# ufukpage/TripleD-Exploring-Depth-Estimation-with-Self-Supervised-Representation-Learning

Measured on AMD Instinct MI355X. Metric: train imgs/sec at KITTI 192x640 bs=12/GPU, higher is better.
Workload: dtype bf16 convs (MFMA) + f32 loss kernels

## Files before the change

### include/tripled_hip.h

```cpp
#ifndef TRIPLED_HIP_H
#define TRIPLED_HIP_H

#include <stddef.h>
#include <stdint.h>

#ifdef __cplusplus
extern "C" {
#endif

#define TD_ABI_VERSION 3
#define TD_MAX_SRC 4

#define TD_OK 0
#define TD_ERR_BAD_ARG (-1)
#define TD_ERR_UNSUPPORTED (-2)
#define TD_ERR_LAUNCH (-3)
#define TD_ERR_WORKSPACE (-4)

typedef void* td_stream_t;

int td_abi_version(void);
const char* td_error_string(int code);
const char* td_last_hip_error(void);

// ... 53 lines not shown

int td_maxpool5_fwd(const void* in, int dtype, int N, int H, int W, int C, void* out, uint8_t* idx,
                    td_stream_t stream);
int td_maxpool5_bwd(const void* grad_out, const uint8_t* idx, int dtype, int N, int H, int W, int C,
                    void* grad_in, td_stream_t stream);
int td_maxpool5_bwd_add(const void* grad_out, const uint8_t* idx, const void* add, int dtype, int N, int H, int W, int C,
                        void* grad_in, td_stream_t stream);

int td_maxpool3s2_fwd(const void* in, int dtype, int N, int H, int W, int C, void* out, uint8_t* idx,
                      td_stream_t stream);
int td_maxpool3s2_bwd(const void* grad_out, const uint8_t* idx, int dtype, int N, int H, int W, int C,
                      void* grad_in, td_stream_t stream);

int td_join_fwd(const void* a, const void* b, const void* tail, int dtype, long long npix, int C0, int C1, int C2,
                void* out, td_stream_t stream);
int td_join_bwd(const void* grad_out, int dtype, long long npix, int C0, int C1, int C2, void* grad_a, void* grad_b,
                void* grad_tail, td_stream_t stream);
int td_join_up2_fwd(const void* a, const void* b_half, const void* tail, int dtype, int N, int H, int W, int C0, int C1,
                    int C2, void* out, td_stream_t stream);
int td_join_up2_bwd(const void* grad_out, int dtype, int N, int H, int W, int C0, int C1, int C2, void* grad_a,
                    void* grad_b_half, void* grad_tail, td_stream_t stream);

long long td_bn_workspace_floats(long long M, int groups, int C);
int td_bn_fwd(const void* x, const void* residual, int dtype, const float* gamma, const float* beta,
              float* running_mean, float* running_var, float momentum, float eps, int relu, long long M, int groups,
              int C, void* y, float* save_mean, float* save_invstd, float* workspace, td_stream_t stream);
int td_bn_bwd(const void* dy, const void* x, const void* y, int dtype, const float* gamma, const float* beta, const float* save_mean,
              const float* save_invstd, int relu, long long M, int groups, int C, void* dx, void* dresidual,
              float* dgamma, float* dbeta, float* workspace, td_stream_t stream);

int td_conv1x1_stat_rows(long long M, int groups, int N);
int td_conv1x1_fwd(const void* x, const void* w, long long M, int groups, int K, int N, int Hi, int Wi, int stride, void* y,
                   float* stat_partials, td_stream_t stream);
int td_conv3x3_fwd(const void* x, const void* w, int B, int groups, int Hi, int Wi, int Cin, int N, int stride, int pad, void* y,
                   float* stat_partials, td_stream_t stream);
long long td_conv3x3_wgrad_workspace_floats(int B, int Ho, int Wo, int C, int N);
int td_conv3x3_wgrad(const void* dy, const void* x, int B, int Ho, int Wo, int C, int N, int pad, int dw_dtype, void* dw,
                     float* workspace, td_stream_t stream);
long long td_conv1x1_wgrad_workspace_floats(long long M, int K, int N);
int td_conv1x1_wgrad(const void* dy, const void* x, long long M, int K, int N, int Hi, int Wi, int stride, int dw_dtype, void* dw,
                     float* workspace, td_stream_t stream);
int td_conv1x1_wgrad_group(int n, const void* const* dy, const void* const* x, const long long* M, const int* K, const int* N,
                           const int* Hi, const int* Wi, const int* stride, const int* dw_dtype, void* const* dw,
                           float* const* workspace, td_stream_t stream);
int td_bn_fwd_from_partials(const void* x, const void* residual, int dtype, const float* gamma, const float* beta,
                            float* running_mean, float* running_var, float momentum, float eps, int relu, long long M,
                            int groups, int C, float* partials, int stat_rows, void* y, float* save_mean,
                            float* save_invstd, td_stream_t stream);

long long td_bias_act_workspace_floats(long long M, int C);
int td_bias_act_fwd(const void* y, const void* bias, int bias_dtype, int dtype, long long M, int C, int act, void* a, td_stream_t stream);
int td_bias_act_bwd(const void* g, const void* a, int dtype, long long M, int C, int act, void* gy, void* dbias, int dbias_dtype,
                    float* workspace, td_stream_t stream);

int td_adam_flat(float* w, const float* grad, float* exp_avg, float* exp_avg_sq, void* lowp, long long n, long long n_lowp,
                 const float* step, const float* lr_dev, float lr_host, double beta1, double beta2, float eps, const float* total_norm,
                 float max_norm, td_stream_t stream);

int td_gather_flat(const void* const* srcs, const long long* dst_offsets, const long long* numels, int n, int src_dtype, float* flat,
                   td_stream_t stream);

int td_bn_partial_rows(long long M, int groups, int C);
int td_bn_fwd_partials(const void* x, int dtype, long long M, int groups, int C, float* partials, td_stream_t stream);
int td_bn_bwd_partials(const void* dy, const void* x, const void* y, int dtype, const float* gamma, const float* beta,
                       const float* save_mean, const float* save_invstd, int relu, long long M, int groups, int C, float* partials,
                       td_stream_t stream);
int td_bn_bwd_from_partials(const void* dy, const void* x, const void* y, int dtype, const float* gamma, const float* beta,
                            const float* save_mean, const float* save_invstd, int relu, long long M, int groups, int C,
                            float* partials, int stat_rows, void* dx, void* dresidual, float* dgamma, float* dbeta,
                            td_stream_t stream);
int td_conv1x1_fwd_bnrelu(const void* z, const void* w, long long M, int groups, int K, int N, float* in_partials, int in_rows,
                          const float* gamma, const float* beta, float* running_mean, float* running_var, float momentum, float eps,
                          float* save_mean, float* save_invstd, void* a_side, void* y, float* stat_partials, td_stream_t stream);
int td_conv1x1_dgrad(const void* dy, const void* w, long long M, int groups, int Cout, int Cin, const void* residual, void* dx,
                     td_stream_t stream);
int td_conv1x1_fwd_sum(const void* x, const void* w, long long M, int K, int N, const void* run_in, void* y, void* run_out,
                       td_stream_t stream);
int td_conv1x1_dgrad_bnsums(const void* dy, const void* w, long long M, int groups, int Cout, int Cin, const void* z,
                            const float* gamma, const float* beta, const float* save_mean, const float* save_invstd, void* dx,
                            float* out_partials, td_stream_t stream);
int td_conv1x1_dgrad_bnbwd(const void* g, const void* z, const void* w, long long M, int groups, int Cout, int Cin, float* in_partials,
                           int in_rows, const float* gamma, const float* beta, const float* save_mean, const float* save_invstd,
                           float* dgamma, float* dbeta, void* dz_side, const void* residual, void* dx, td_stream_t stream);

int td_bn_sync_fwd_sums(const void* x, int dtype, long long M, int groups, int C, float* sums, float* workspace,
                        td_stream_t stream);
int td_bn_sync_fwd_apply(const void* x, const void* residual, int dtype, const float* sums, const float* count,
                         const float* gamma, const float* beta, float* running_mean, float* running_var, float momentum,
                         float eps, int relu, long long M, int groups, int C, void* y, float* save_mean,
                         float* save_invstd, td_stream_t stream);
int td_bn_sync_bwd_sums(const void* dy, const void* x, const void* y, int dtype, const float* gamma, const float* beta,
                        const float* save_mean, const float* save_invstd, int relu, long long M, int groups, int C,
                        float* sums, float* workspace, td_stream_t stream);
int td_bn_sync_bwd_dx(const void* dy, const void* x, const void* y, int dtype, const float* local_sums,
                      const float* global_sums, const float* count, const float* gamma, const float* beta,
                      const float* save_mean, const float* save_invstd, int relu, long long M, int groups, int C,
                      void* dx, void* dresidual, float* dgamma, float* dbeta, float* coef, td_stream_t stream);

int td_edge_weights(const float* img, int B, int h, int w, float a, const float* scale6, float* Wt,
                    td_stream_t stream);
int td_featreg_num_blocks(int B, int h, int w, int C);
int td_featreg_fwd(const void* feat, int dtype, const float* Wt, int B, int h, int w, int C,
                   float* partial, td_stream_t stream);
int td_featreg_bwd(const void* feat, int dtype, const float* Wt, const float* gscale, int B, int h, int w,
                   int C, void* grad, td_stream_t stream);

// ... 139 lines not shown
```

### tripled-exploring-depth-estimation-with-self-supervised-representation-learning_amd/csrc/td_biasact.hip

```cpp
#include <hip/hip_bf16.h>

#include "td_common.h"
#include "td_vec8.h"

namespace td {

template <int ACT>
__device__ __forceinline__ float ba_fwd(float z) {
  if (ACT == 1) return z > 0.f ? z : expm1f(z);
  if (ACT == 2) return z > 0.f ? z : 0.01f * z;
  return z;
}
template <int ACT>
__device__ __forceinline__ float ba_bwd(float g, float a) {
  if (ACT == 1) return a > 0.f ? g : g * (a + 1.f);
  if (ACT == 2) return a > 0.f ? g : 0.01f * g;
  return g;
}

template <typename T, int ACT>
__global__ __launch_bounds__(TD_THREADS) void bias_act_fwd_kernel(const T* __restrict__ y, const void* __restrict__ bias, int bias_bf16,
                                                                  long long nvec, int cvec, T* __restrict__ a) {
  const long long stride = (long long)gridDim.x * TD_THREADS;
  long long i = (long long)blockIdx.x * TD_THREADS + threadIdx.x;
  const int cg = (int)(i % cvec);
  float b[8];
#pragma unroll
  for (int e = 0; e < 8; ++e)
    b[e] = !bias ? 0.f : bias_bf16 ? bf2f(reinterpret_cast<const unsigned short*>(bias)[cg * 8 + e]) : reinterpret_cast<const float*>(bias)[cg * 8 + e];
  for (; i < nvec; i += stride) {
    float v[8];
    load8(y + i * 8, v);
#pragma unroll
    for (int e = 0; e < 8; ++e) v[e] = ba_fwd<ACT>(v[e] + b[e]);
    store8(a + i * 8, v);
  }
}

template <typename T, int ACT>
__global__ __launch_bounds__(TD_THREADS) void bias_act_bwd_kernel(const T* __restrict__ g, const T* __restrict__ a, long long nvec, int cvec,
                                                                  T* __restrict__ gy, float* __restrict__ partial) {
  __shared__ float red[TD_THREADS][9];
  const long long stride = (long long)gridDim.x * TD_THREADS;
  long long i = (long long)blockIdx.x * TD_THREADS + threadIdx.x;
  float s[8];
#pragma unroll
  for (int e = 0; e < 8; ++e) s[e] = 0.f;
  for (; i < nvec; i += stride) {
    float vg[8], va[8];
    load8(g + i * 8, vg);
    if (ACT != 0) load8(a + i * 8, va);
#pragma unroll
    for (int e = 0; e < 8; ++e) {
      vg[e] = ba_bwd<ACT>(vg[e], ACT != 0 ? va[e] : 0.f);
      s[e] += vg[e];
    }
    if (ACT != 0) store8(gy + i * 8, vg);
  }
#pragma unroll
  for (int e = 0; e < 8; ++e) red[threadIdx.x][e] = s[e];
  __syncthreads();
  const int C = cvec * 8;
  if ((int)threadIdx.x < C) {
    const int c = threadIdx.x, cg = c >> 3, e = c & 7;
    float t = 0.f;
    for (int j = cg; j < TD_THREADS; j += cvec) t += red[j][e];
    partial[(size_t)blockIdx.x * C + c] = t;
  }
}

template <typename T>
// ... 79 lines not shown
```

### tripled-exploring-depth-estimation-with-self-supervised-representation-learning_amd/hostside/mono/model/networks.py

```python
import os

import numpy as np
import torch
import torch.nn as nn
import torch.nn.functional as F



FUSED_BN_OFF = bool(os.environ.get("TD_NO_FUSED_BN"))


def _ops():
    from tripled_amd import ops
    return ops


def _dense_cl(x):
    if x.is_cuda and x.dim() == 4 and x.shape[1] % 8 == 0 and x.dtype in (torch.float32, torch.bfloat16) \
            and not x.is_contiguous(memory_format=torch.channels_last) and x.stride(1) == 1:
        return x.contiguous(memory_format=torch.channels_last)
    return x


def _fell_back(site, x, why=""):
# ... 506 lines not shown
            y = F.conv2d(x, w, b)
        ctx.save_for_backward(x, w)
        ctx.has_bias = b is not None
        return y

    @staticmethod
    def backward(ctx, gy):
        x, w = ctx.saved_tensors
        with torch.backends.cudnn.flags(enabled=True, benchmark=False):
            gx, gw, gb = torch.ops.aten.convolution_backward(gy, x, w, [w.shape[0]] if ctx.has_bias else None, [1, 1], [0, 0], [1, 1],
                                                              False, [0, 0], 1, [True, True, ctx.has_bias])
        return gx, gw, (gb if ctx.has_bias else None)


class _KeepChannels(torch.autograd.Function):

    @staticmethod
    def forward(ctx, y, c):
        ctx.pad = y.shape[1] - c
        return y.narrow(1, 0, c)

    @staticmethod
    def backward(ctx, g):
        return F.pad(g, (0, 0, 0, 0, 0, ctx.pad)), None


FUSED_BIAS_ACT_OFF = bool(os.environ.get("TD_NO_FUSED_BIAS_ACT"))
FUSED_CRP_OFF = bool(os.environ.get("TD_NO_FUSED_CRP"))


def _activate(y, act):
    if act == "elu":
        return F.elu(y, inplace=True)
    if act == "leaky_relu":
        return F.leaky_relu(y)
    return y


def _conv2d_guarded(x, w, b, act=None):
    if x.is_cuda and x.shape[1] <= 16 and w.shape[0] <= 16 and x.shape[3] > 1024 and torch.backends.cudnn.benchmark:
        if torch.is_autocast_enabled():
            dt = torch.get_autocast_dtype("cuda")
            x, w, b = x.to(dt), w.to(dt), (b.to(dt) if b is not None else None)
        return _activate(_ConvImmediate.apply(x, w, b), act)
    if (act is not None or b is not None) and x.is_cuda and not FUSED_BIAS_ACT_OFF and torch.is_grad_enabled() \
            and torch.is_autocast_enabled() and torch.get_autocast_dtype("cuda") == torch.bfloat16:
        xb = x if x.dtype == torch.bfloat16 else x.to(torch.bfloat16)
        wb = w if w.dtype == torch.bfloat16 else w.to(torch.bfloat16)
        if _ops().conv_bias_act_supported(xb, wb, b, act):
            return _ops().conv_bias_act(xb, wb, b, act)
    return _activate(F.conv2d(x, w, b), act)


class Conv3x3(nn.Module):

    def __init__(self, in_channels, out_channels, use_refl=True):
        super().__init__()
        self.use_refl = use_refl
        self.pad = nn.ReflectionPad2d(1) if use_refl else nn.ZeroPad2d(1)
        self.conv = nn.Conv2d(int(in_channels), int(out_channels), 3)

    def _pad_input(self, x):
        x = _dense_cl(x)
        if self.use_refl and x.shape[1] % 8 == 0 and x.dtype in (torch.float32, torch.bfloat16) \
                and x.is_contiguous(memory_format=torch.channels_last) and x.shape[2] >= 2 and x.shape[3] >= 2:
            from tripled_amd import ops
            return ops.reflpad1(x)
        if self.use_refl:
            _fell_back("Conv3x3.pad", x)
        return self.pad(x)

    def forward(self, x, act=None):
        low_precision = x.is_cuda and (x.dtype == torch.bfloat16 or torch.is_autocast_enabled())
        if not low_precision or os.environ.get("TD_NO_CHANNEL_PAD"):
            return _activate(self.conv(self._pad_input(x) if x.is_cuda else self.pad(x)), act)
        w, b = self.conv.weight, self.conv.bias
        cout, cin = w.shape[0], w.shape[1]
        cin_p, cout_p = _round8(cin), _round8(cout)
        if cin_p == cin and cout_p == cout and x.shape[1] == cin:
            return _conv2d_guarded(self._pad_input(x), w, b, act)
        if x.shape[1] == cin and cin_p != cin:
            x = torch.cat((x, x.new_zeros(x.shape[0], cin_p - cin, x.shape[2], x.shape[3])), 1)
        if x.shape[1] != cin_p:
            raise ValueError("Conv3x3 expects %d (or pre-padded %d) input channels, got %d" % (cin, cin_p, x.shape[1]))
        if not x.is_contiguous(memory_format=torch.channels_last):
            x = x.contiguous(memory_format=torch.channels_last)
        w = F.pad(w, (0, 0, 0, 0, 0, cin_p - cin, 0, cout_p - cout))
        if b is not None and cout_p != cout:
            b = F.pad(b, (0, cout_p - cout))
        if cout_p != cout:
            return _activate(_KeepChannels.apply(_conv2d_guarded(self._pad_input(x), w, b), cout), act)
        return _conv2d_guarded(self._pad_input(x), w, b, act)

    def forward_up(self, x, act=None):
        w, b = self.conv.weight, self.conv.bias
        cout, cin = w.shape[0], w.shape[1]
        x = _dense_cl(x)
        low_precision = x.is_cuda and (x.dtype == torch.bfloat16 or torch.is_autocast_enabled())
        if (self.use_refl and x.is_cuda and x.shape[1] == cin and cin % 8 == 0 and (cout % 8 == 0 or low_precision)
                and x.dtype in (torch.float32, torch.bfloat16) and x.is_contiguous(memory_format=torch.channels_last)
                and not os.environ.get("TD_NO_FUSED_UPSAMPLE")):
            cout_p = _round8(cout)
            if cout_p != cout:
                w = F.pad(w, (0, 0, 0, 0, 0, 0, 0, cout_p - cout))
                b = F.pad(b, (0, cout_p - cout)) if b is not None else None
            if cout_p != cout:
                return _activate(_KeepChannels.apply(_conv2d_guarded(_ops().up2_reflpad1(x), w, b), cout), act)
            return _conv2d_guarded(_ops().up2_reflpad1(x), w, b, act)
        _fell_back("Conv3x3.forward_up", x)
        return self.forward(upsample(x), act)


class Conv5x5(nn.Module):
    def __init__(self, in_channels, out_channels, use_refl=True):
        super().__init__()
        self.pad = nn.ReflectionPad2d(2) if use_refl else nn.ZeroPad2d(2)
        self.conv = nn.Conv2d(int(in_channels), int(out_channels), 5)

    def forward(self, x):
        return self.conv(self.pad(x))


class ConvBlock(nn.Module):
    def __init__(self, in_channels, out_channels):
        super().__init__()
        self.conv = Conv3x3(in_channels, out_channels)
        self.nonlin = nn.ELU(inplace=True)

    def forward(self, x):
        return self.conv(x, act="elu")

    def forward_up(self, x):
        return self.conv.forward_up(x, act="elu")


class CRPBlock(nn.Module):

    def __init__(self, in_planes, out_planes, n_stages):
        super().__init__()
        for i in range(n_stages):
            setattr(self, "{}_{}".format(i + 1, "pointwise"),
                    Conv1x1(in_planes if i == 0 else out_planes, out_planes, False))
        self.stride = 1
        self.n_stages = n_stages
        self.maxpool = nn.MaxPool2d(kernel_size=5, stride=1, padding=2)

    def _pool(self, t):
        if t.is_cuda and t.is_contiguous(memory_format=torch.channels_last) and t.shape[1] % 8 == 0 \
                and t.dtype in (torch.float32, torch.bfloat16):
            from tripled_amd import ops
            return ops.maxpool5(t)
        _fell_back("CRPBlock.maxpool", t)
        return self.maxpool(t)

    def _fused(self, x):
        if FUSED_CRP_OFF or _FP8_1X1[0] or not (self.training and x.is_cuda and torch.is_grad_enabled()):
            return None
        if not (torch.is_autocast_enabled() and torch.get_autocast_dtype("cuda") == torch.bfloat16):
            return None
        convs = [getattr(self, "{}_{}".format(i + 1, "pointwise")).conv for i in range(self.n_stages)]
        if any(c.bias is not None for c in convs):
# ... 204 lines not shown
```

### tripled-exploring-depth-estimation-with-self-supervised-representation-learning_amd/native.py

```python
import ctypes
import os

import torch

from . import dispatch

_HERE = os.path.dirname(os.path.abspath(__file__))
LIB_PATH = os.path.join(_HERE, "lib", "libtripled_hip.so")

TD_MAX_SRC = 4

_PTRARR = ctypes.POINTER(ctypes.c_void_p)
_I, _F, _P = ctypes.c_int, ctypes.c_float, ctypes.c_void_p
_LLARR = ctypes.POINTER(ctypes.c_longlong)
_IARR = ctypes.POINTER(ctypes.c_int)
ABI_VERSION = 3

SIGNATURES = {
    "td_abi_version": (_I, []),
    "td_error_string": (ctypes.c_char_p, [_I]),
    "td_last_hip_error": (ctypes.c_char_p, []),
    "td_photo_num_blocks": (_I, [_I, _I, _I]),
    "td_photo_bwd_num_blocks": (_I, [_I, _I, _I]),
    "td_photo_identity": (_I, [_P, _PTRARR, _I, _I, _I, _I, _P, _P, _PTRARR, _P]),
    "td_photo_fwd": (_I, [_P, _PTRARR, _I, _P, _P, _P, _P, _P, _I, _I, _I, _I, _I, _F, _F, _P, _P, _P, _P, _P, _P]),
    "td_photo_bwd": (_I, [_P, _PTRARR, _P, _PTRARR, _I, _P, _P, _P, _P, _P, _I, _P, _F, _I, _I, _I, _I, _I, _F, _F, _P, _P, _P]),
    "td_pack_rgbx": (_I, [_P, _I, _I, _I, _P, _P]),
    "td_upsample_adjoint": (_I, [_P, _I, _I, _I, _I, _I, _P, _I, _P]),
    "td_upsample_adjoint_planes": (_I, [_P, _I, _I, _I, _I, _I, _I, _P, _I, _P]),
    "td_reduce_dP": (_I, [_P, _I, _I, _I, _I, _P, _P]),
    "td_sum_scaled": (_I, [_P, _I, _F, _P, _P]),
    "td_area_downsample": (_I, [_P, _I, _I, _I, _I, _I, _I, _P, _P]),
    "td_smooth_num_blocks": (_I, [_I, _I, _I]),
    "td_smooth_fwd": (_I, [_P, _P, _I, _I, _I, _I, _P, _P, _P]),
    "td_smooth_finish": (_I, [_P, _I, _I, _I, _F, _P, _P]),
    "td_smooth_bwd": (_I, [_P, _P, _P, _I, _I, _I, _I, _P, _F, _P, _P, _P, _I, _P]),
    "td_maxpool5_fwd": (_I, [_P, _I, _I, _I, _I, _I, _P, _P, _P]),
    "td_maxpool5_bwd": (_I, [_P, _P, _I, _I, _I, _I, _I, _P, _P]),
    "td_maxpool5_bwd_add": (_I, [_P, _P, _P, _I, _I, _I, _I, _I, _P, _P]),
    "td_conv1x1_fwd_sum": (_I, [_P, _P, ctypes.c_longlong, _I, _I, _P, _P, _P, _P]),
    "td_maxpool3s2_fwd": (_I, [_P, _I, _I, _I, _I, _I, _P, _P, _P]),
    "td_maxpool3s2_bwd": (_I, [_P, _P, _I, _I, _I, _I, _I, _P, _P]),
    "td_join_fwd": (_I, [_P, _P, _P, _I, ctypes.c_longlong, _I, _I, _I, _P, _P]),
    "td_join_bwd": (_I, [_P, _I, ctypes.c_longlong, _I, _I, _I, _P, _P, _P, _P]),
    "td_join_up2_fwd": (_I, [_P, _P, _P, _I, _I, _I, _I, _I, _I, _I, _P, _P]),
    "td_join_up2_bwd": (_I, [_P, _I, _I, _I, _I, _I, _I, _I, _P, _P, _P, _P]),
    "td_bn_workspace_floats": (ctypes.c_longlong, [ctypes.c_longlong, _I, _I]),
    "td_bn_fwd": (_I, [_P, _P, _I, _P, _P, _P, _P, _F, _F, _I, ctypes.c_longlong, _I, _I, _P, _P, _P, _P, _P]),
    "td_conv1x1_stat_rows": (_I, [ctypes.c_longlong, _I, _I]),
    "td_conv1x1_fwd": (_I, [_P, _P, ctypes.c_longlong, _I, _I, _I, _I, _I, _I, _P, _P, _P]),
    "td_conv3x3_fwd": (_I, [_P, _P, _I, _I, _I, _I, _I, _I, _I, _I, _P, _P, _P]),
    "td_conv3x3_wgrad_workspace_floats": (ctypes.c_longlong, [_I, _I, _I, _I, _I]),
    "td_conv3x3_wgrad": (_I, [_P, _P, _I, _I, _I, _I, _I, _I, _I, _P, _P, _P]),
    "td_conv1x1_wgrad_workspace_floats": (ctypes.c_longlong, [ctypes.c_longlong, _I, _I]),
    "td_conv1x1_wgrad": (_I, [_P, _P, ctypes.c_longlong, _I, _I, _I, _I, _I, _I, _P, _P, _P]),
    "td_conv1x1_wgrad_group": (_I, [_I, _PTRARR, _PTRARR, _LLARR, _IARR, _IARR, _IARR, _IARR, _IARR, _IARR, _PTRARR, _PTRARR, _P]),
    "td_bn_fwd_from_partials": (_I, [_P, _P, _I, _P, _P, _P, _P, _F, _F, _I, ctypes.c_longlong, _I, _I, _P, _I, _P, _P, _P, _P]),
    "td_bias_act_workspace_floats": (ctypes.c_longlong, [ctypes.c_longlong, _I]),
    "td_bias_act_fwd": (_I, [_P, _P, _I, _I, ctypes.c_longlong, _I, _I, _P, _P]),
    "td_bias_act_bwd": (_I, [_P, _P, _I, ctypes.c_longlong, _I, _I, _P, _P, _I, _P, _P]),
    "td_gather_flat": (_I, [_PTRARR, _LLARR, _LLARR, _I, _I, _P, _P]),
    "td_adam_flat": (_I, [_P, _P, _P, _P, _P, ctypes.c_longlong, ctypes.c_longlong, _P, _P, _F, ctypes.c_double, ctypes.c_double, _F, _P, _F, _P]),
    "td_bn_partial_rows": (_I, [ctypes.c_longlong, _I, _I]),
    "td_bn_fwd_partials": (_I, [_P, _I, ctypes.c_longlong, _I, _I, _P, _P]),
    "td_bn_bwd_partials": (_I, [_P, _P, _P, _I, _P, _P, _P, _P, _I, ctypes.c_longlong, _I, _I, _P, _P]),
    "td_bn_bwd_from_partials": (_I, [_P, _P, _P, _I, _P, _P, _P, _P, _I, ctypes.c_longlong, _I, _I, _P, _I, _P, _P, _P, _P, _P]),
    "td_conv1x1_fwd_bnrelu": (_I, [_P, _P, ctypes.c_longlong, _I, _I, _I, _P, _I, _P, _P, _P, _P, _F, _F, _P, _P, _P, _P, _P, _P]),
    "td_conv1x1_dgrad": (_I, [_P, _P, ctypes.c_longlong, _I, _I, _I, _P, _P, _P]),
    "td_conv1x1_dgrad_bnsums": (_I, [_P, _P, ctypes.c_longlong, _I, _I, _I, _P, _P, _P, _P, _P, _P, _P, _P]),
    "td_conv1x1_dgrad_bnbwd": (_I, [_P, _P, _P, ctypes.c_longlong, _I, _I, _I, _P, _I, _P, _P, _P, _P, _P, _P, _P, _P, _P, _P]),
    "td_bn_bwd": (_I, [_P, _P, _P, _I, _P, _P, _P, _P, _I, ctypes.c_longlong, _I, _I, _P, _P, _P, _P, _P, _P]),
    "td_edge_weights": (_I, [_P, _I, _I, _I, _F, ctypes.POINTER(ctypes.c_float), _P, _P]),
    "td_featreg_num_blocks": (_I, [_I, _I, _I, _I]),
    "td_featreg_fwd": (_I, [_P, _I, _P, _I, _I, _I, _I, _P, _P]),
    "td_featreg_bwd": (_I, [_P, _I, _P, _P, _I, _I, _I, _I, _P, _P]),
    "td_recon_num_tasks": (_I, [_I, _I, _I]),
    "td_recon_fwd": (_I, [_P, _P, _P, _I, _I, _I, _P, _P]),
    "td_recon_bwd": (_I, [_P, _P, _P, _P, _I, _I, _I, _P, _P]),
    "td_reflpad1_fwd": (_I, [_P, _I, _I, _I, _I, _I, _P, _P]),
    "td_reflpad1_bwd": (_I, [_P, _I, _I, _I, _I, _I, _P, _P]),
    "td_up2_reflpad1_fwd": (_I, [_P, _I, _I, _I, _I, _I, _P, _P]),
    "td_up2_reflpad1_bwd": (_I, [_P, _I, _I, _I, _I, _I, _P, _P]),
    "td_featwarp_num_blocks": (_I, [_I, _I, _I]),
    "td_featwarp_fwd": (_I, [_P, _PTRARR, _I, _I, _P, _P, _P, _I, _I, _I, _I, _I, _I, _F, _F, _P, _P, _P]),
    "td_featwarp_bwd": (_I, [_P, _PTRARR, _I, _I, _P, _P, _P, _P, _P, _F, _I, _I, _I, _I, _I, _I, _F, _F, _P, _PTRARR,
                             _P, _P, _P]),
    "td_featwarp_dsrc_finish": (_I, [_P, _P, _F, _I, ctypes.c_longlong, _I, _P, _P]),
    "td_reduce_partials": (_I, [_P, _I, _I, _I, _P, _P]),
    "td_bn_sync_fwd_sums": (_I, [_P, _I, ctypes.c_longlong, _I, _I, _P, _P, _P]),
    "td_bn_sync_fwd_apply": (_I, [_P, _P, _I, _P, _P, _P, _P, _P, _P, _F, _F, _I, ctypes.c_longlong, _I, _I, _P, _P, _P, _P]),
    "td_bn_sync_bwd_sums": (_I, [_P, _P, _P, _I, _P, _P, _P, _P, _I, ctypes.c_longlong, _I, _I, _P, _P, _P]),
    "td_bn_sync_bwd_dx": (_I, [_P, _P, _P, _I, _P, _P, _P, _P, _P, _P, _P, _I, ctypes.c_longlong, _I, _I, _P, _P, _P, _P, _P, _P]),
    "td_fp8_num_blocks": (_I, [ctypes.c_longlong]),
    "td_fp8_amax_partials": (_I, [_P, _I, ctypes.c_longlong, _P, _P]),
    "td_fp8_quantize": (_I, [_P, _I, ctypes.c_longlong, _P, _P, _P, _P]),
    "td_color_jitter": (_I, [_P, _P, _I, _I, _I, _P, _P, _P, _P]),
    "td_l1map_fwd": (_I, [_P, _I, _LLARR, _P, _I, _I, _I, _I, _F, _P, _P]),
    "td_l1map_bwd": (_I, [_P, _I, _LLARR, _P, _P, _I, _I, _I, _I, _F, _P, _P]),
    "td_rgb2lab": (_I, [_P, _I, _I, _I, _F, _F, _F, _P, _P]),
    "td_pose_fwd": (_I, [_P, _P, _IARR, _P, _I, _I, _P, _P, _P]),
    "td_pose_bwd": (_I, [_P, _P, _IARR, _P, _I, _I, _P, _P, _P, _P, _P]),
    "td_infer_preprocess": (_I, [_P, _I, _I, _I, _I, _I, _I, _P, _P]),
    "td_disp_postprocess": (_I, [_P, _I, _I, _I, _I, _I, _I, _I, _F, _F, _F, _P, _P, _P]),
    "td_colorize": (_I, [_P, _I, ctypes.c_longlong, _P, _P, _P, _P, _P]),
    "td_eval_depth_workspace_bytes": (ctypes.c_longlong, [_I, _I, _I]),
    "td_eval_depth": (_I, [_P, _I, _I, _I, _I, _F, _F, _P, _I, _I, _P, _P, _F, _F, _I, _P, ctypes.c_longlong, _P, _P, _P]),
    "td_masked_median_workspace_bytes": (ctypes.c_longlong, [_I]),
    "td_masked_median": (_I, [_P, _I, ctypes.c_longlong, _P, ctypes.c_longlong, _P, _P, _P]),
    "td_pose_pairs_u8": (_I, [_P, _I, _I, _I, _I, _I, _I, _P, ctypes.c_longlong, _P]),
    "td_odom_trajectory": (_I, [_P, _I, _I, _P, _P]),
    "td_odom_snippet_ate": (_I, [_P, _I, _P, _I, _I, _P, _P]),
    "td_odom_sequence_errors": (_I, [_P, _P, _I, ctypes.POINTER(ctypes.c_double), _I, _I, _I, _P, _P, _P, _P, _P]),
    "td_lanczos_resize_u8": (_I, [_P, _P, _IARR, _P, ctypes.c_longlong, _IARR, _I, _I, _I, _I, _I, _I, _P, _P, _P]),
# ... 152 lines not shown
```

### tripled-exploring-depth-estimation-with-self-supervised-representation-learning_amd/ops.py

```python
import ctypes
import os
import types

import torch

from . import native
from .native import call

_CL = torch.channels_last


def _f32c(t):
    if t.dtype != torch.float32:
        t = t.float()
    return t if t.is_contiguous() else t.contiguous()


def _f32(n, like):
    return torch.empty(n, device=like.device, dtype=torch.float32)


def _cl(t, dtype=None):
    return (t if dtype is None else t.to(dtype)).contiguous(memory_format=_CL)

# ... 816 lines not shown
        x, y, hole = ctx.saved_tensors
        B, _, h, w = x.shape
        dx = torch.empty_like(x)
        call("td_recon_bwd", x, y, hole, _f32c(g.reshape(1)), B, h, w, dx)
        return dx, None, None


def masked_reconstruction_sum(pred, target, hole):
    if pred.shape[2] < 3 or pred.shape[3] < 3:
        raise native.NativeLibraryError("masked_reconstruction_sum needs h, w >= 3")
    pred = pred.float().contiguous()
    return _ReconSum.apply(pred, _f32c(target.detach()), _f32c(hole.detach()))


def _pad_fwd(name, x, Ho, Wo):
    N, C, H, W = x.shape
    out = _empty_cl(N, C, Ho, Wo, x)
    call(name, x, x.dtype, N, H, W, C, out)
    return out


def _pad_bwd(name, g, H, W):
    N, C = g.shape[:2]
    g = _cl(g)
    gin = _empty_cl(N, C, H, W, g)
    call(name, g, g.dtype, N, H, W, C, gin)
    return gin


class _ReflPad1(torch.autograd.Function):
    @staticmethod
    def forward(ctx, x):
        return _pad_fwd("td_reflpad1_fwd", x, x.shape[2] + 2, x.shape[3] + 2)

    @staticmethod
    def backward(ctx, g):
        return _pad_bwd("td_reflpad1_bwd", g, g.shape[2] - 2, g.shape[3] - 2)


class _Up2ReflPad1(torch.autograd.Function):
    @staticmethod
    def forward(ctx, x):
        return _pad_fwd("td_up2_reflpad1_fwd", x, 2 * x.shape[2] + 2, 2 * x.shape[3] + 2)

    @staticmethod
    def backward(ctx, g):
        return _pad_bwd("td_up2_reflpad1_bwd", g, (g.shape[2] - 2) // 2, (g.shape[3] - 2) // 2)


def up2_reflpad1_supported(x):
    return _cl_tensor(x, 8)


def up2_reflpad1(x):
    if not up2_reflpad1_supported(x):
        raise native.NativeLibraryError("up2_reflpad1 needs a channels_last f32/bf16 HIP tensor with C % 8 == 0")
    return _Up2ReflPad1.apply(x)


def reflpad1_supported(x):
    return _cl_tensor(x, 8) and x.shape[2] >= 2 and x.shape[3] >= 2


def reflpad1(x):
    if not reflpad1_supported(x):
        raise native.NativeLibraryError("reflpad1 needs a channels_last f32/bf16 HIP tensor with C % 8 == 0")
    return _ReflPad1.apply(x)


class _FeatureWarpLoss(torch.autograd.Function):
    @staticmethod
    def forward(ctx, tgt_f, disp, P, invK, min_depth, max_depth, *src_f):
        B, C, h, w = tgt_f.shape
        hs, ws = disp.shape[2], disp.shape[3]
        dev = tgt_f.device
        n_src = len(src_f)
        disp = _f32c(disp)
        P = _f32c(P)
        argmin = torch.empty(B, h, w, device=dev, dtype=torch.uint8)
        nblk = native.load().td_featwarp_num_blocks(B, h, w)
        partial, loss = _f32(nblk, tgt_f), _f32(1, tgt_f)
        call("td_featwarp_fwd", tgt_f, src_f, n_src, tgt_f.dtype, disp, P, invK, B, h, w, C, hs, ws, float(min_depth),
             float(max_depth), argmin, partial)
        inv_count = 1.0 / float(B * h * w)
        call("td_sum_scaled", partial, nblk, inv_count, loss)
        ctx.save_for_backward(tgt_f, disp, P, invK, argmin, *src_f)
        ctx.meta = (min_depth, max_depth, inv_count, nblk)
        ctx.mark_non_differentiable(argmin)
        return loss.reshape(()), argmin

    @staticmethod
    def backward(ctx, g, _g_idx):
        tgt_f, disp, P, invK, argmin, *src_f = ctx.saved_tensors
        min_depth, max_depth, inv_count, nblk = ctx.meta
        B, C, h, w = tgt_f.shape
        hs, ws = disp.shape[2], disp.shape[3]
        dev = tgt_f.device
        n_src = len(src_f)
        gs = _f32c(g.reshape(1))
        d_tgt = torch.empty_like(tgt_f, memory_format=_CL)
        d_src32 = [torch.zeros((B, h, w, C), device=dev, dtype=torch.int32) for _ in src_f]
        d_up = torch.empty(B, h, w, device=dev, dtype=torch.float32)
        dP_part = torch.empty(nblk, n_src * 12, device=dev, dtype=torch.float32)
        call("td_featwarp_bwd", tgt_f, src_f, n_src, tgt_f.dtype, disp, P, invK, argmin, gs, inv_count, B, h, w, C, hs, ws,
             float(min_depth), float(max_depth), d_tgt, d_src32, d_up, dP_part)
        d_disp = torch.empty_like(disp)
# ... 158 lines not shown
```

Baseline: 434.4.

## Add MFMA narrow-channel 3x3 conv kernel fusing reflect pad, upsample, bias and activation

Adds a custom HIP kernel for 3x3 convolutions with few channels (Cin 16/32, Cout 8/16/32). It reads reflect-padded or 2x-upsampled reflect-padded input on the fly, runs bf16 MFMA over row strips with rolling accumulators, and applies bias and activation in the epilogue. A matching dgrad kernel uses zero-pad-2 with flipped weights. This removes the separate pad/upsample tensors and the generic conv launch for the decoder's narrow layers. Weight gradients still use aten convolution_backward, and bias is added after rounding the accumulator to bf16.

```diff
diff --git a/include/tripled_hip.h b/include/tripled_hip.h
--- a/include/tripled_hip.h
+++ b/include/tripled_hip.h
@@ -129,6 +129,11 @@
 int td_bias_act_fwd(const void* y, const void* bias, int bias_dtype, int dtype, long long M, int C, int act, void* a, td_stream_t stream);
 int td_bias_act_bwd(const void* g, const void* a, int dtype, long long M, int C, int act, void* gy, void* dbias, int dbias_dtype,
                     float* workspace, td_stream_t stream);
+
+int td_conv3x3_narrow_fwd(const void* x, const void* w, int w_channels_last, const void* bias, int bias_dtype, int B, int H, int W,
+                          int Cin, int Cout, int mode, int act, void* y, td_stream_t stream);
+int td_conv3x3_narrow_dgrad(const void* gy, const void* w, int w_channels_last, int B, int H, int W, int Cin, int Cout, void* dxp,
+                            td_stream_t stream);
 
 int td_adam_flat(float* w, const float* grad, float* exp_avg, float* exp_avg_sq, void* lowp, long long n, long long n_lowp,
                  const float* step, const float* lr_dev, float lr_host, double beta1, double beta2, float eps, const float* total_norm,
diff --git a/tripled-exploring-depth-estimation-with-self-supervised-representation-learning_amd/csrc/td_act.h b/tripled-exploring-depth-estimation-with-self-supervised-representation-learning_amd/csrc/td_act.h
--- /dev/null
+++ b/tripled-exploring-depth-estimation-with-self-supervised-representation-learning_amd/csrc/td_act.h
@@ -0,0 +1,19 @@
+#pragma once
+#include <hip/hip_runtime.h>
+
+namespace td {
+
+template <int ACT>
+__device__ __forceinline__ float ba_fwd(float z) {
+  if (ACT == 1) return z > 0.f ? z : expm1f(z);
+  if (ACT == 2) return z > 0.f ? z : 0.01f * z;
+  return z;
+}
+template <int ACT>
+__device__ __forceinline__ float ba_bwd(float g, float a) {
+  if (ACT == 1) return a > 0.f ? g : g * (a + 1.f);
+  if (ACT == 2) return a > 0.f ? g : 0.01f * g;
+  return g;
+}
+
+}
diff --git a/tripled-exploring-depth-estimation-with-self-supervised-representation-learning_amd/csrc/td_biasact.hip b/tripled-exploring-depth-estimation-with-self-supervised-representation-learning_amd/csrc/td_biasact.hip
--- a/tripled-exploring-depth-estimation-with-self-supervised-representation-learning_amd/csrc/td_biasact.hip
+++ b/tripled-exploring-depth-estimation-with-self-supervised-representation-learning_amd/csrc/td_biasact.hip
@@ -1,22 +1,10 @@
 #include <hip/hip_bf16.h>
 
+#include "td_act.h"
 #include "td_common.h"
 #include "td_vec8.h"
 
 namespace td {
-
-template <int ACT>
-__device__ __forceinline__ float ba_fwd(float z) {
-  if (ACT == 1) return z > 0.f ? z : expm1f(z);
-  if (ACT == 2) return z > 0.f ? z : 0.01f * z;
-  return z;
-}
-template <int ACT>
-__device__ __forceinline__ float ba_bwd(float g, float a) {
-  if (ACT == 1) return a > 0.f ? g : g * (a + 1.f);
-  if (ACT == 2) return a > 0.f ? g : 0.01f * g;
-  return g;
-}
 
 template <typename T, int ACT>
 __global__ __launch_bounds__(TD_THREADS) void bias_act_fwd_kernel(const T* __restrict__ y, const void* __restrict__ bias, int bias_bf16,
diff --git a/tripled-exploring-depth-estimation-with-self-supervised-representation-learning_amd/csrc/td_conv3x3_narrow.hip b/tripled-exploring-depth-estimation-with-self-supervised-representation-learning_amd/csrc/td_conv3x3_narrow.hip
--- /dev/null
+++ b/tripled-exploring-depth-estimation-with-self-supervised-representation-learning_amd/csrc/td_conv3x3_narrow.hip
@@ -0,0 +1,233 @@
+#include <hip/hip_bf16.h>
+
+#include "td_act.h"
+#include "td_common.h"
+#include "td_vec8.h"
+
+namespace td {
+
+typedef __attribute__((ext_vector_type(8))) __bf16 cn_bf16x8;
+typedef __attribute__((ext_vector_type(4))) float cn_f32x4;
+
+constexpr int CN_REFLECT1 = 0, CN_UP2_REFLECT1 = 1, CN_ZERO2 = 2;
+constexpr int CN_THREADS = 256;
+constexpr int CN_ROWS = 8;
+
+struct CnGeom {
+  int Hi, Wi, Ho, Wo;
+  int ctiles, rtiles;
+  long long strips;
+  int N, Nw;
+  long long wsn, wsc, wsy, wsx;
+  int act, bias_bf16;
+};
+
+template <int K, int NT, int MODE>
+__global__ __launch_bounds__(CN_THREADS) void conv3x3_narrow_kernel(const unsigned short* __restrict__ x, const unsigned short* __restrict__ w,
+                                                                    const void* __restrict__ bias, unsigned short* __restrict__ y, CnGeom g) {
+  constexpr int S = (3 * K + 31) / 32;
+  constexpr int WF = 3 * S * NT;
+  __shared__ __attribute__((aligned(16))) unsigned short wl[WF * 512];
+
+  for (int e = threadIdx.x; e < WF * 512; e += CN_THREADS) {
+    const int j = e & 7, l = (e >> 3) & 63, f = e >> 9;
+    const int t = f % NT, s = (f / NT) % S, ky = f / (NT * S);
+    const int n = 16 * t + (l & 15), kk = 32 * s + 8 * (l >> 4) + j;
+    const int kx = kk / K, c = kk - kx * K;
+    unsigned short v = 0;
+    if (n < g.Nw && kx < 3) v = w[n * g.wsn + c * g.wsc + ky * g.wsy + kx * g.wsx];
+    wl[e] = v;
+  }
+  __syncthreads();
+  const int lane = threadIdx.x & 63;
+  const long long strip = (long long)blockIdx.x * (CN_THREADS / 64) + __builtin_amdgcn_readfirstlane(threadIdx.x >> 6);
+  if (strip >= g.strips) return;
+  cn_bf16x8 wf[3][S][NT];
+#pragma unroll
+  for (int ky = 0; ky < 3; ++ky)
+#pragma unroll
+    for (int s = 0; s < S; ++s)
+#pragma unroll
+      for (int t = 0; t < NT; ++t)
+        wf[ky][s][t] = __builtin_bit_cast(cn_bf16x8, *reinterpret_cast<const uint4*>(wl + (((ky * S + s) * NT + t) * 64 + lane) * 8));
+
+  const int ct = (int)(strip % g.ctiles);
+  const long long sr = strip / g.ctiles;
+  const int rt = (int)(sr % g.rtiles), b = (int)(sr / g.rtiles);
+  const int r0 = rt * CN_ROWS;
+  const int rows = g.Ho - r0 < CN_ROWS ? g.Ho - r0 : CN_ROWS;
+  const int col = lane & 15, q = lane >> 4;
+  const int ocol = ct * 16 + col;
+  const int oc = ocol < g.Wo ? ocol : g.Wo - 1;
+
+  int coff[S];
+  bool cok[S];
+#pragma unroll
+  for (int s = 0; s < S; ++s) {
+    const int k0 = 32 * s + 8 * q;
+    int kx = k0 / K;
+    kx = kx > 2 ? 2 : kx;
+    const int ch = k0 % K;
+    int sc;
+    cok[s] = true;
+    if (MODE == CN_REFLECT1) sc = reflect1(oc - 1 + kx, g.Wi);
+    else if (MODE == CN_UP2_REFLECT1) sc = reflect1(oc - 1 + kx, 2 * g.Wi) >> 1;
+    else {
+      sc = oc - 2 + kx;
+      cok[s] = sc >= 0 && sc < g.Wi;
+      sc = sc < 0 ? 0 : (sc >= g.Wi ? g.Wi - 1 : sc);
+    }
+    coff[s] = (sc * K + ch) * 2;
+  }
+  const unsigned char* xb = reinterpret_cast<const unsigned char*>(x) + (long long)b * g.Hi * g.Wi * K * 2;
+  const long long xrow = (long long)g.Wi * K * 2;
+
+  auto load_row = [&](int i, uint4 (&fr)[S]) {
+    int rr;
+    bool rok = true;
+    if (MODE == CN_REFLECT1) rr = reflect1(r0 - 1 + i, g.Hi);
+    else if (MODE == CN_UP2_REFLECT1) rr = reflect1(r0 - 1 + i, 2 * g.Hi) >> 1;
+    else {
+      rr = r0 - 2 + i;
+      rok = rr >= 0 && rr < g.Hi;
+      rr = rr < 0 ? 0 : (rr >= g.Hi ? g.Hi - 1 : rr);
+    }
+    const unsigned char* p = xb + rr * xrow;
+#pragma unroll
+    for (int s = 0; s < S; ++s) {
+      fr[s] = *reinterpret_cast<const uint4*>(p + coff[s]);
+      if (MODE == CN_ZERO2) {
+        const bool ok = rok && cok[s];
+        fr[s].x = ok ? fr[s].x : 0u; fr[s].y = ok ? fr[s].y : 0u; fr[s].z = ok ? fr[s].z : 0u; fr[s].w = ok ? fr[s].w : 0u;
+      }
+    }
+  };
+
+  float bv[NT][4];
+#pragma unroll
+  for (int t = 0; t < NT; ++t)
+#pragma unroll
+    for (int e = 0; e < 4; ++e) {
+      const int n = 16 * t + 4 * q + e;
+      bv[t][e] = (!bias || n >= g.N) ? 0.f
+                 : g.bias_bf16 ? bf2f(reinterpret_cast<const unsigned short*>(bias)[n]) : reinterpret_cast<const float*>(bias)[n];
+    }
+  unsigned short* yb = y + ((long long)b * g.Ho * g.Wo + ocol) * g.N + 4 * q;
+  const bool store_ok = ocol < g.Wo;
+
+  auto store_row = [&](int r, const cn_f32x4 (&a)[NT]) {
+#pragma unroll
+    for (int t = 0; t < NT; ++t) {
+      float v[4];
+#pragma unroll
+      for (int e = 0; e < 4; ++e) {
+        const float z = bf2f(f2bf(a[t][e])) + bv[t][e];
+        v[e] = g.act == 1 ? ba_fwd<1>(z) : g.act == 2 ? ba_fwd<2>(z) : z;
+      }
+      uint2 p;
+      p.x = (unsigned)f2bf(v[0]) | ((unsigned)f2bf(v[1]) << 16);
+      p.y = (unsigned)f2bf(v[2]) | ((unsigned)f2bf(v[3]) << 16);
+      if (store_ok && 16 * t + 4 * q < g.N) *reinterpret_cast<uint2*>(yb + (long long)r * g.Wo * g.N + 16 * t) = p;
+    }
+  };
+
+  cn_f32x4 a0[NT], a1[NT], a2[NT];
+#pragma unroll
+  for (int t = 0; t < NT; ++t) a0[t] = a1[t] = a2[t] = cn_f32x4{0.f, 0.f, 0.f, 0.f};
+  uint4 cur[S], nxt[S];
+  load_row(0, cur);
+  const int nit = rows + 2;
+  auto step = [&](int i, cn_f32x4 (&k2)[NT], cn_f32x4 (&k1)[NT], cn_f32x4 (&k0)[NT]) {
+    load_row(i + 1, nxt);
+#pragma unroll
+    for (int t = 0; t < NT; ++t) k0[t] = cn_f32x4{0.f, 0.f, 0.f, 0.f};
+#pragma unroll
+    for (int s = 0; s < S; ++s) {
+      const cn_bf16x8 f = __builtin_bit_cast(cn_bf16x8, cur[s]);
+#pragma unroll
+      for (int t = 0; t < NT; ++t) {
+        k2[t] = __builtin_amdgcn_mfma_f32_16x16x32_bf16(wf[2][s][t], f, k2[t], 0, 0, 0);
+        k1[t] = __builtin_amdgcn_mfma_f32_16x16x32_bf16(wf[1][s][t], f, k1[t], 0, 0, 0);
+        k0[t] = __builtin_amdgcn_mfma_f32_16x16x32_bf16(wf[0][s][t], f, k0[t], 0, 0, 0);
+      }
+    }
+    if (i >= 2) store_row(r0 + i - 2, k2);
+#pragma unroll
+    for (int s = 0; s < S; ++s) cur[s] = nxt[s];
+  };
+  for (int i = 0; i < nit; i += 3) {
+    step(i, a1, a2, a0);
+    if (i + 1 < nit) step(i + 1, a2, a0, a1);
+    if (i + 2 < nit) step(i + 2, a0, a1, a2);
+  }
+}
+
+template <int K, int NT, int MODE>
+static int cn_launch(const void* x, const void* w, const void* bias, void* y, const CnGeom& g, hipStream_t st) {
+  const long long blocks = (g.strips + CN_THREADS / 64 - 1) / (CN_THREADS / 64);
+  if (blocks > 0x7fffffffll) return TD_ERR_UNSUPPORTED;
+  hipLaunchKernelGGL((conv3x3_narrow_kernel<K, NT, MODE>), dim3((unsigned)blocks), dim3(CN_THREADS), 0, st, (const unsigned short*)x,
+                     (const unsigned short*)w, bias, (unsigned short*)y, g);
+  return TD_OK;
+}
+
+template <int MODE>
+static int cn_dispatch(int K, int nt, const void* x, const void* w, const void* bias, void* y, const CnGeom& g, hipStream_t st) {
+#define TD_CN(KK, TT) if (K == KK && nt == TT) return cn_launch<KK, TT, MODE>(x, w, bias, y, g, st);
+  if constexpr (MODE == CN_ZERO2) { TD_CN(8, 1) TD_CN(8, 2) }
+  TD_CN(16, 1) TD_CN(16, 2) TD_CN(32, 1) TD_CN(32, 2)
+#undef TD_CN
+  return TD_ERR_UNSUPPORTED;
+}
+
+static void cn_strips(CnGeom& g, int B) {
+  g.ctiles = (g.Wo + 15) / 16;
+  g.rtiles = (g.Ho + CN_ROWS - 1) / CN_ROWS;
+  g.strips = (long long)B * g.rtiles * g.ctiles;
+}
+
+}
+
+extern "C" int td_conv3x3_narrow_fwd(const void* x, const void* w, int w_channels_last, const void* bias, int bias_dtype, int B, int H, int W,
+                                     int Cin, int Cout, int mode, int act, void* y, td_stream_t stream) {
+  if (!x || !w || !y || B <= 0 || H <= 0 || W <= 0) return TD_ERR_BAD_ARG;
+  if (mode != td::CN_REFLECT1 && mode != td::CN_UP2_REFLECT1) return TD_ERR_BAD_ARG;
+  if (act < 0 || act > 2 || (bias && bias_dtype != TD_DTYPE_BF16 && bias_dtype != TD_DTYPE_F32)) return TD_ERR_BAD_ARG;
+  if ((Cin != 16 && Cin != 32) || (Cout != 8 && Cout != 16 && Cout != 32)) return TD_ERR_UNSUPPORTED;
+  if (mode == td::CN_REFLECT1 && (H < 2 || W < 2)) return TD_ERR_UNSUPPORTED;
+  const int up = mode == td::CN_UP2_REFLECT1 ? 2 : 1;
+  if ((long long)B * H * W * up * up >= (1ll << 31) / 64) return TD_ERR_UNSUPPORTED;
+  td::CnGeom g = {};
+  g.Hi = H; g.Wi = W; g.Ho = up * H; g.Wo = up * W;
+  td::cn_strips(g, B);
+  g.N = Cout; g.Nw = Cout;
+  if (w_channels_last) { g.wsn = 9ll * Cin; g.wsc = 1; g.wsy = 3ll * Cin; g.wsx = Cin; }
+  else { g.wsn = 9ll * Cin; g.wsc = 9; g.wsy = 3; g.wsx = 1; }
+  g.act = act; g.bias_bf16 = bias_dtype == TD_DTYPE_BF16;
+  hipStream_t st = (hipStream_t)stream;
+  const int nt = Cout > 16 ? 2 : 1;
+  const int rc = mode == td::CN_REFLECT1 ? td::cn_dispatch<td::CN_REFLECT1>(Cin, nt, x, w, bias, y, g, st)
+                                         : td::cn_dispatch<td::CN_UP2_REFLECT1>(Cin, nt, x, w, bias, y, g, st);
+  if (rc != TD_OK) return rc;
+  return td::record_launch_error(hipGetLastError(), "td_conv3x3_narrow_fwd");
+}
+
+extern "C" int td_conv3x3_narrow_dgrad(const void* gy, const void* w, int w_channels_last, int B, int H, int W, int Cin, int Cout, void* dxp,
+                                       td_stream_t stream) {
+  if (!gy || !w || !dxp || B <= 0 || H <= 0 || W <= 0) return TD_ERR_BAD_ARG;
+  if ((Cin != 16 && Cin != 32) || (Cout != 8 && Cout != 16 && Cout != 32)) return TD_ERR_UNSUPPORTED;
+  if ((long long)B * (H + 2) * (W + 2) >= (1ll << 31) / 64) return TD_ERR_UNSUPPORTED;
+  td::CnGeom g = {};
+  g.Hi = H; g.Wi = W; g.Ho = H + 2; g.Wo = W + 2;
+  td::cn_strips(g, B);
+  g.N = Cin; g.Nw = Cin;
+  long long sn, sc, sy, sx;
+  if (w_channels_last) { sn = 9ll * Cin; sc = 1; sy = 3ll * Cin; sx = Cin; }
+  else { sn = 9ll * Cin; sc = 9; sy = 3; sx = 1; }
+  g.wsn = sc; g.wsc = sn; g.wsy = -sy; g.wsx = -sx;
+  const unsigned short* wp = (const unsigned short*)w + 2 * sy + 2 * sx;
+  g.act = 0; g.bias_bf16 = 0;
+  const int rc = td::cn_dispatch<td::CN_ZERO2>(Cout, Cin > 16 ? 2 : 1, gy, wp, nullptr, dxp, g, (hipStream_t)stream);
+  if (rc != TD_OK) return rc;
+  return td::record_launch_error(hipGetLastError(), "td_conv3x3_narrow_dgrad");
+}
diff --git a/tripled-exploring-depth-estimation-with-self-supervised-representation-learning_amd/hostside/mono/model/networks.py b/tripled-exploring-depth-estimation-with-self-supervised-representation-learning_amd/hostside/mono/model/networks.py
--- a/tripled-exploring-depth-estimation-with-self-supervised-representation-learning_amd/hostside/mono/model/networks.py
+++ b/tripled-exploring-depth-estimation-with-self-supervised-representation-learning_amd/hostside/mono/model/networks.py
@@ -582,6 +582,19 @@
     return _activate(F.conv2d(x, w, b), act)
 
 
+def _conv3x3_narrow(x, w, b, act, mode):
+    if not (x.is_cuda and x.dtype == torch.bfloat16 and x.dim() == 4 and x.shape[1] in (16, 32) and w.shape[0] in (8, 16, 32)
+            and w.shape[1] == x.shape[1]) or FUSED_BIAS_ACT_OFF or not torch.is_grad_enabled() or not torch.is_autocast_enabled():
+        return None
+    ops = _ops()
+    if ops.NARROW_CONV3X3_OFF or x.shape[3] * (2 if mode == "up2_reflect1" else 1) + 2 > ops.NARROW_MAX_PADDED_WIDTH:
+        return None
+    wb = w if w.dtype == torch.bfloat16 else w.to(torch.bfloat16)
+    if ops.conv3x3_narrow_supported(x, wb, b, act, mode):
+        return ops.conv3x3_narrow(x, wb, b, act, mode)
+    return None
+
+
 class Conv3x3(nn.Module):
 
     def __init__(self, in_channels, out_channels, use_refl=True):
@@ -608,7 +621,8 @@
         cout, cin = w.shape[0], w.shape[1]
         cin_p, cout_p = _round8(cin), _round8(cout)
         if cin_p == cin and cout_p == cout and x.shape[1] == cin:
-            return _conv2d_guarded(self._pad_input(x), w, b, act)
+            y = _conv3x3_narrow(_dense_cl(x), w, b, act, "reflect1") if self.use_refl else None
+            return y if y is not None else _conv2d_guarded(self._pad_input(x), w, b, act)
         if x.shape[1] == cin and cin_p != cin:
             x = torch.cat((x, x.new_zeros(x.shape[0], cin_p - cin, x.shape[2], x.shape[3])), 1)
         if x.shape[1] != cin_p:
@@ -619,7 +633,8 @@
         if b is not None and cout_p != cout:
             b = F.pad(b, (0, cout_p - cout))
         if cout_p != cout:
-            return _activate(_KeepChannels.apply(_conv2d_guarded(self._pad_input(x), w, b), cout), act)
+            y = _conv3x3_narrow(x, w, b, None, "reflect1") if self.use_refl else None
+            return _activate(_KeepChannels.apply(y if y is not None else _conv2d_guarded(self._pad_input(x), w, b), cout), act)
         return _conv2d_guarded(self._pad_input(x), w, b, act)
 
     def forward_up(self, x, act=None):
@@ -635,8 +650,10 @@
                 w = F.pad(w, (0, 0, 0, 0, 0, 0, 0, cout_p - cout))
                 b = F.pad(b, (0, cout_p - cout)) if b is not None else None
             if cout_p != cout:
-                return _activate(_KeepChannels.apply(_conv2d_guarded(_ops().up2_reflpad1(x), w, b), cout), act)
-            return _conv2d_guarded(_ops().up2_reflpad1(x), w, b, act)
+                y = _conv3x3_narrow(x, w, b, None, "up2_reflect1")
+                return _activate(_KeepChannels.apply(y if y is not None else _conv2d_guarded(_ops().up2_reflpad1(x), w, b), cout), act)
+            y = _conv3x3_narrow(x, w, b, act, "up2_reflect1")
+            return y if y is not None else _conv2d_guarded(_ops().up2_reflpad1(x), w, b, act)
         _fell_back("Conv3x3.forward_up", x)
         return self.forward(upsample(x), act)
 
diff --git a/tripled-exploring-depth-estimation-with-self-supervised-representation-learning_amd/native.py b/tripled-exploring-depth-estimation-with-self-supervised-representation-learning_amd/native.py
--- a/tripled-exploring-depth-estimation-with-self-supervised-representation-learning_amd/native.py
+++ b/tripled-exploring-depth-estimation-with-self-supervised-representation-learning_amd/native.py
@@ -59,6 +59,8 @@
     "td_bias_act_workspace_floats": (ctypes.c_longlong, [ctypes.c_longlong, _I]),
     "td_bias_act_fwd": (_I, [_P, _P, _I, _I, ctypes.c_longlong, _I, _I, _P, _P]),
     "td_bias_act_bwd": (_I, [_P, _P, _I, ctypes.c_longlong, _I, _I, _P, _P, _I, _P, _P]),
+    "td_conv3x3_narrow_fwd": (_I, [_P, _P, _I, _P, _I, _I, _I, _I, _I, _I, _I, _I, _P, _P]),
+    "td_conv3x3_narrow_dgrad": (_I, [_P, _P, _I, _I, _I, _I, _I, _I, _P, _P]),
     "td_gather_flat": (_I, [_PTRARR, _LLARR, _LLARR, _I, _I, _P, _P]),
     "td_adam_flat": (_I, [_P, _P, _P, _P, _P, ctypes.c_longlong, ctypes.c_longlong, _P, _P, _F, ctypes.c_double, ctypes.c_double, _F, _P, _F, _P]),
     "td_bn_partial_rows": (_I, [ctypes.c_longlong, _I, _I]),
diff --git a/tripled-exploring-depth-estimation-with-self-supervised-representation-learning_amd/ops.py b/tripled-exploring-depth-estimation-with-self-supervised-representation-learning_amd/ops.py
--- a/tripled-exploring-depth-estimation-with-self-supervised-representation-learning_amd/ops.py
+++ b/tripled-exploring-depth-estimation-with-self-supervised-representation-learning_amd/ops.py
@@ -892,6 +892,88 @@
     return _cl_tensor(x, 8)
 
 
+NARROW_CONV3X3_OFF = bool(os.environ.get("TD_NO_NARROW_CONV3X3"))
+NARROW_MODES = {"reflect1": 0, "up2_reflect1": 1}
+NARROW_MAX_PADDED_WIDTH = 1024
+_NARROW_LAYERS = frozenset((m, ci, co) for m in NARROW_MODES for ci in (16, 32) for co in (8, 16, 32))
+NARROW_DISPATCH = {"fwd": _NARROW_LAYERS, "dgrad": _NARROW_LAYERS, "wgrad": frozenset()}
+
+
+def _bf16_autocast():
+    return torch.is_autocast_enabled() and torch.get_autocast_dtype("cuda") == torch.bfloat16
+
+
+def _narrow_weight_layout(w):
+    if w.is_contiguous():
+        return 0
+    return 1 if w.is_contiguous(memory_format=_CL) else None
+
+
+class _Conv3x3Narrow(torch.autograd.Function):
+
+    @staticmethod
+    def forward(ctx, x, w, b, act, mode):
+        B, Cin, H, W = x.shape
+        Cout, up = w.shape[0], 2 if mode == "up2_reflect1" else 1
+        y = _empty_cl(B, Cout, up * H, up * W, x)
+        call("td_conv3x3_narrow_fwd", x, w, _narrow_weight_layout(w), b, b.dtype if b is not None else 0, B, H, W, Cin, Cout,
+             NARROW_MODES[mode], ACT_CODES[act], y)
+        ctx.save_for_backward(x, w, b, y if act is not None else None)
+        ctx.act, ctx.mode = act, mode
+        return y
+
+    @staticmethod
+    def backward(ctx, g):
+        x, w, b, a = ctx.saved_tensors
+        B, C, Ho, Wo = g.shape
+        Cin, H, W = x.shape[1:]
+        g = _cl(g, w.dtype)
+        M = B * Ho * Wo
+        gy = torch.empty_like(g, memory_format=_CL) if ctx.act is not None else g
+        db = torch.empty_like(b) if b is not None and ctx.needs_input_grad[2] else None
+        if ctx.act is not None or db is not None:
+            ws = _f32(native.load().td_bias_act_workspace_floats(M, C), g)
+            call("td_bias_act_bwd", g, a, g.dtype, M, C, ACT_CODES[ctx.act], gy if ctx.act is not None else None, db,
+                 db.dtype if db is not None else 0, ws)
+        pad = "td_up2_reflpad1" if ctx.mode == "up2_reflect1" else "td_reflpad1"
+        key = (ctx.mode, Cin, C)
+        need_dx, need_dw = ctx.needs_input_grad[:2]
+        own_dx = need_dx and key in NARROW_DISPATCH["dgrad"]
+        dxp = dw = None
+        if (need_dx and not own_dx) or need_dw:
+            xp = _pad_fwd(pad + "_fwd", x, Ho + 2, Wo + 2) if need_dw else _empty_cl(B, Cin, Ho + 2, Wo + 2, x)
+            dxp, dw, _ = torch.ops.aten.convolution_backward(gy, xp, w, None, [1, 1], [0, 0], [1, 1], False, [0, 0], 1,
+                                                             [need_dx and not own_dx, need_dw, False])
+        if own_dx:
+            dxp = _empty_cl(B, Cin, Ho + 2, Wo + 2, x)
+            call("td_conv3x3_narrow_dgrad", gy, w, _narrow_weight_layout(w), B, Ho, Wo, Cin, C, dxp)
+        dx = _pad_bwd(pad + "_bwd", dxp, H, W) if need_dx else None
+        return dx, dw, db, None, None
+
+
+def conv3x3_narrow_supported(x, w, b, act, mode):
+    if NARROW_CONV3X3_OFF or act not in ACT_CODES or mode not in NARROW_MODES or not torch.is_grad_enabled() or not _bf16_autocast():
+        return False
+    if not (x.is_cuda and x.dim() == 4 and x.dtype == torch.bfloat16 and x.is_contiguous(memory_format=_CL)):
+        return False
+    if not (w.dim() == 4 and w.dtype == torch.bfloat16 and tuple(w.shape[1:]) == (x.shape[1], 3, 3) and _narrow_weight_layout(w) is not None):
+        return False
+    if b is not None and not (b.dtype in native.DTYPE_CODES and b.dim() == 1 and b.shape[0] == w.shape[0] and b.is_contiguous()):
+        return False
+    up = 2 if mode == "up2_reflect1" else 1
+    H, W = x.shape[2], x.shape[3]
+    if (mode == "reflect1" and (H < 2 or W < 2)) or up * W + 2 > NARROW_MAX_PADDED_WIDTH or x.shape[0] * up * H * up * W >= (1 << 25):
+        return False
+    return (mode, x.shape[1], w.shape[0]) in NARROW_DISPATCH["fwd"]
+
+
+def conv3x3_narrow(x, w, b, act=None, mode="reflect1"):
+    if not conv3x3_narrow_supported(x, w, b, act, mode):
+        raise native.NativeLibraryError("conv3x3_narrow needs a bf16 channels_last HIP activation under bf16 autocast, Cin in {16, 32}, "
+                                        "Cout in {8, 16, 32} and a padded width of at most %d" % NARROW_MAX_PADDED_WIDTH)
+    return _Conv3x3Narrow.apply(x, w, b, act, mode)
+
+
 def up2_reflpad1(x):
     if not up2_reflpad1_supported(x):
         raise native.NativeLibraryError("up2_reflpad1 needs a channels_last f32/bf16 HIP tensor with C % 8 == 0")
```

Result: no change. 438.4, median of 6 (+0.9%).
